# zubair-irshad/NeO-360

Measured on AMD Instinct MI355X. Metric: rays/sec (128 samples/ray) + PSNR vs ref, 640x480, higher is better.
Workload: dtype f32 (fp16-MFMA products of hi/lo-split fp32 operands, fp32 accumulate)

## Files before the change

neo-360_amd/csrc/mlp_tp_hp.hip:

```cpp
#include <hip/hip_fp16.h>

#include <algorithm>
#include <cstdlib>
#include <type_traits>

#include "tp_hp_layout.h"

#ifndef NEO_TP_WPS
#define NEO_TP_WPS 2
#endif
#ifndef NEO_TP_RING
#define NEO_TP_RING 3
#endif
#ifndef NEO_TP_STAGGER_DEFAULT
#define NEO_TP_STAGGER_DEFAULT 0
#endif
#ifndef NEO_TP_XSTREAM
#define NEO_TP_XSTREAM 2
#endif
#ifndef NEO_TP_ABLATE
#define NEO_TP_ABLATE 0
#endif
#define TP_SYNC() __syncthreads()
#ifndef NEO_TP_TRACE
#define NEO_TP_TRACE 0
#endif
#if NEO_TP_TRACE
__device__ unsigned long long g_tp_trace[16];
#define TP_MARK(k) do { const unsigned long long now_ = __builtin_amdgcn_s_memtime(); tr_[k] += now_ - tlast_; tlast_ = now_; } while (0)
#else
#define TP_MARK(k) do { } while (0)
#endif

namespace neo {

namespace {

using namespace hp;
constexpr int RING = NEO_TP_RING;

template <int PE_C, bool CULL = false, bool DENS = false>
__global__ __launch_bounds__(256, NEO_TP_WPS) void k_tp_mlp_hp(TpMlpHDev m, const float* __restrict__ proj, TpScene sc,
                                                             TpViews views, const float* __restrict__ rays_o,
                                                             const float* __restrict__ rays_d,
                                                             const float* __restrict__ viewdirs,
                                                             const float* __restrict__ tvals,
                                                             const float* __restrict__ far_arr, int R, int N, int chunk,
                                                             uint32_t* __restrict__ flags, float4* __restrict__ out, int stagger,
                                                             const float* __restrict__ dirsum) {
    extern __shared__ __attribute__((aligned(16))) float smem[];
    if (stagger > 0 && blockIdx.x >= 256u && blockIdx.x < 512u)
        for (int i = 0; i < stagger; i += 100) __builtin_amdgcn_s_sleep(100);
    _Float16* hbase = reinterpret_cast<_Float16*>(smem + tp::OFF_ACT);
    const HT act{hbase, hbase + TM * 128};
    auto xbuf = [&](int b) { return HT{hbase + b * (2 * TM * 64), hbase + b * (2 * TM * 64) + TM * 64}; };
    auto fbuf = [&](int b) { return smem + tp::OFF_ACT + b * (TM * 64); };
    _Float16* dbase = reinterpret_cast<_Float16*>(smem + tp::OFF_DIR);
    const HT dsm{dbase, dbase + TM * 32};
    const tp::Scratch S = tp::carve(smem);
    int* loc_off = S.loc_off;
    float* loc_w = S.loc_w;
    int* pl_off = S.pl_off;
    float* pl_w = S.pl_w;
    float* cam_enc = S.cam_enc;

    LaneCtx L;
    L.init();
    int tid = threadIdx.x;
    const long P = tp::launch_points<CULL>(sc, R, N);
    const long tile0 = tp::xcd_tile<CULL>(blockIdx.x, (P + TM - 1) / TM) * TM;
    if (tile0 >= P) return;
    const h8* wp = reinterpret_cast<const h8*>(m.wpack);
    constexpr int KSX = ks_x(PE_C);
    constexpr int NPE = PE_C == 3 ? 1 : 2;

#if NEO_TP_TRACE
    unsigned long long tr_[8] = {0, 0, 0, 0, 0, 0, 0, 0}, tlast_ = __builtin_amdgcn_s_memtime();
#endif
    tp::point_setup<PE_C>(S, tid, tile0, P, N, R, chunk, rays_o, rays_d, viewdirs, tvals, far_arr, flags, false, sc.grid_w, sc.grid_first, sc.grid_pw, sc.grid_ph, CULL ? sc.cull_map : nullptr, CULL ? 0 : sc.quad);
    float* dens_w = smem + tp::OFF_DENSW;
    if (tid < 128) dens_w[tid] = m.heads[HD_DW + tid];
    float* lbias_w = smem + tp::LDS_WORDS;
    for (int i = tid; i < 768; i += 256) lbias_w[i] = m.bias[i];
    for (int i = tid; i < HD_RB + 3; i += 256) lbias_w[768 + i] = m.heads[i];
    const float* lbias = lbias_w;
    const float* lheads = lbias_w + 768;
    float* dsum = smem + tp::OFF_DIR;
    TP_SYNC();
    if constexpr (!DENS) {
        const int p = tid >> 2, f0 = (tid & 3) << 3;
        const int dray = __float_as_int(S.vdir_world[p * 4 + 3]);
        const f32x4 s0 = *reinterpret_cast<const f32x4*>(dirsum + (long)dray * 32 + f0);
        const f32x4 s1 = *reinterpret_cast<const f32x4*>(dirsum + (long)dray * 32 + f0 + 4);
#pragma unroll
        for (int j = 0; j < 8; ++j) dsum[p * 32 + ((f0 + j) ^ (p & 31))] = j < 4 ? s0[j] : s1[j - 4];
        TP_SYNC();
    }
    TP_MARK(0);

    f32x16 hsum[2];
#pragma unroll
    for (int r = 0; r < 16; ++r) { hsum[0][r] = 0.f; hsum[1][r] = 0.f; }
    [[maybe_unused]] const int nts_1[1] = {L.wv};
    const int vnt = L.wv & 1, vmt = L.wv >> 1;

#pragma unroll 1
    for (int v = 0; v < sc.nv; ++v) {
        asm volatile("" : "+v"(tid));
        L.lane = tid & 63;
        L.half = L.lane >> 5;
        L.l31 = L.lane & 31;
        L.key = L.lane & 15;
// ... 390 lines not shown
            if constexpr (g == 13) {
                TP_SYNC();
                store_tile_h<true>(y, act, vnt, vmt, L);
            }
            __builtin_amdgcn_sched_barrier(0);
        });
        TP_SYNC();
    }
    {
        const int pt = L.wv * 16 + (L.lane >> 2), part = L.lane & 3;
        [[maybe_unused]] float r = 0.f, g = 0.f, b = 0.f;
        if constexpr (!DENS) {
            const float* wr = lheads + HD_RW;
#pragma unroll
            for (int c = 0; c < 2; ++c) {
                const int chunk_i = part * 2 + ((c + part) & 1);
                const int o = chunk_off<128>(pt, chunk_i);
                const h8 vh = *reinterpret_cast<const h8*>(act.hi + o);
                const h8 vl = *reinterpret_cast<const h8*>(act.lo + o);
#pragma unroll
                for (int e = 0; e < 8; ++e) {
                    const float h = (float)vh[e] + (float)vl[e];
                    r += h * wr[chunk_i * 8 + e];
                    g += h * wr[64 + chunk_i * 8 + e];
                    b += h * wr[128 + chunk_i * 8 + e];
                }
            }
            r += __shfl_xor(r, 1, 64); r += __shfl_xor(r, 2, 64);
            g += __shfl_xor(g, 1, 64); g += __shfl_xor(g, 2, 64);
            b += __shfl_xor(b, 1, 64); b += __shfl_xor(b, 2, 64);
        }
        range_commit(L, m.flags);
        const long gv = tile0 + pt;
        const long gi = tp::launch_point(gv, N, R, CULL ? 0 : sc.quad, sc.grid_w, sc.grid_first, sc.grid_pw, sc.grid_ph);
        if (part == 0 && gv < P) {
            if constexpr (DENS)
                out[gi] = make_float4(0.0f, 0.0f, 0.0f, density_act(raw_sigma));
            else
                out[gi] = make_float4(colour_act(r + lheads[HD_RB]), colour_act(g + lheads[HD_RB + 1]),
                                      colour_act(b + lheads[HD_RB + 2]), density_act(raw_sigma));
        }
    }
#if NEO_TP_TRACE
    TP_MARK(6);
    if (threadIdx.x == 0) {
#pragma unroll
        for (int k = 0; k < 7; ++k) atomicAdd(&g_tp_trace[k], tr_[k]);
        atomicAdd(&g_tp_trace[7], 1ull);
    }
#endif
}

__global__ void k_tp_dirsum(const float* __restrict__ viewdirs, int R, TpViews views, int nv, float* __restrict__ out) {
    const int r = blockIdx.x * blockDim.x + threadIdx.x;
    if (r >= R) return;
    const float dx = viewdirs[r * 3], dy = viewdirs[r * 3 + 1], dz = viewdirs[r * 3 + 2];
    float acc[27];
#pragma unroll
    for (int f = 0; f < 27; ++f) acc[f] = 0.0f;
    for (int v = 0; v < nv; ++v) {
        const float* rot = views.rot[v];
        const float dc[3] = {rot[0] * dx + rot[1] * dy + rot[2] * dz, rot[3] * dx + rot[4] * dy + rot[5] * dz,
                             rot[6] * dx + rot[7] * dy + rot[8] * dz};
#pragma unroll
        for (int a = 0; a < 3; ++a) acc[a] += dc[a];
#pragma unroll
        for (int k = 0; k < 4; ++k)
// ... 122 lines not shown
                          hipStream_t s, int channels, int in_ch, int first_chunk) {
    if (texels <= 0) return;
    const dim3 grid((unsigned)((texels + 63) / 64));
    const f32x4* wx = reinterpret_cast<const f32x4*>(wpack_f32_stage_x);
    if (channels == 128 && in_ch == 512)
        hipLaunchKernelGGL((k_tp_preproject<1, 64>), grid, dim3(256), 0, s, latent_cl, wx, kc_x, texels, proj, first_chunk);
    else if (in_ch == 512)
        hipLaunchKernelGGL((k_tp_preproject<2, 64>), grid, dim3(256), 0, s, latent_cl, wx, kc_x, texels, proj, first_chunk);
    else
        hipLaunchKernelGGL((k_tp_preproject<2, 16>), grid, dim3(256), 0, s, latent_cl, wx, kc_x, texels, proj, first_chunk);
}

void launch_tp_dirsum(const float* viewdirs, int R, const TpViews& views, int nv, float* dirsum, hipStream_t s) {
    if (R <= 0) return;
    hipLaunchKernelGGL(k_tp_dirsum, dim3((unsigned)((R + 255) / 256)), dim3(256), 0, s, viewdirs, R, views, nv, dirsum);
}

void launch_tp_mlp_hp(int input_ch, const TpMlpHDev& m, const float* proj, const TpScene& sc, const TpViews& views,
                      const float* rays_o, const float* rays_d, const float* viewdirs, const float* tvals,
                      const float* far, int R, int N, int chunk, uint32_t* flags, float* out, const float* dirsum,
                      hipStream_t s, bool density_only) {
    const long P = (long)R * N;
    if (P <= 0) return;
    static int stagger = -1;
    if (stagger < 0) {
        const char* e = getenv("NEO_TP_STAGGER");
        stagger = e ? atoi(e) : NEO_TP_STAGGER_DEFAULT;
    }
    static size_t lds_pad = ~size_t(0);
    if (lds_pad == ~size_t(0)) {
        const char* e = getenv("NEO_TP_LDS_PAD");
        lds_pad = e ? (size_t)atol(e) : 0;
    }
    const size_t lds = (tp::LDS_WORDS + 768 + 336) * sizeof(float) + lds_pad;
    if (lds > 65536) {
        (void)hipFuncSetAttribute(reinterpret_cast<const void*>(k_tp_mlp_hp<3>), hipFuncAttributeMaxDynamicSharedMemorySize, (int)lds);
        (void)hipFuncSetAttribute(reinterpret_cast<const void*>(k_tp_mlp_hp<4>), hipFuncAttributeMaxDynamicSharedMemorySize, (int)lds);
        (void)hipFuncSetAttribute(reinterpret_cast<const void*>(k_tp_mlp_hp<4, true>), hipFuncAttributeMaxDynamicSharedMemorySize, (int)lds);
        (void)hipFuncSetAttribute(reinterpret_cast<const void*>(k_tp_mlp_hp<3, true>), hipFuncAttributeMaxDynamicSharedMemorySize, (int)lds);
        (void)hipFuncSetAttribute(reinterpret_cast<const void*>(k_tp_mlp_hp<3, false, true>), hipFuncAttributeMaxDynamicSharedMemorySize, (int)lds);
        (void)hipFuncSetAttribute(reinterpret_cast<const void*>(k_tp_mlp_hp<4, false, true>), hipFuncAttributeMaxDynamicSharedMemorySize, (int)lds);
        (void)hipFuncSetAttribute(reinterpret_cast<const void*>(k_tp_mlp_hp<4, true, true>), hipFuncAttributeMaxDynamicSharedMemorySize, (int)lds);
    }
    const long tiles = tp::xcd_grid((P + TM - 1) / TM);
    const bool dens = density_only && !(sc.cull_map && input_ch == 3);
    if (dens) {
    } else if (!sc.cull_map && input_ch == 3)
        hipLaunchKernelGGL(k_tp_mlp_hp<3>, dim3((unsigned)tiles), dim3(256), lds, s, m, proj, sc, views, rays_o, rays_d,
                           viewdirs, tvals, far, R, N, chunk, flags, reinterpret_cast<float4*>(out), stagger, dirsum);
    else if (sc.cull_map && input_ch != 3)
        hipLaunchKernelGGL((k_tp_mlp_hp<4, true>), dim3((unsigned)tiles), dim3(256), lds, s, m, proj, sc, views, rays_o, rays_d,
                           viewdirs, tvals, far, R, N, chunk, flags, reinterpret_cast<float4*>(out), stagger, dirsum);
    else if (!sc.cull_map)
        hipLaunchKernelGGL(k_tp_mlp_hp<4>, dim3((unsigned)tiles), dim3(256), lds, s, m, proj, sc, views, rays_o, rays_d,
                           viewdirs, tvals, far, R, N, chunk, flags, reinterpret_cast<float4*>(out), stagger, dirsum);
    else
        hipLaunchKernelGGL((k_tp_mlp_hp<3, true>), dim3((unsigned)tiles), dim3(256), lds, s, m, proj, sc, views, rays_o, rays_d,
                           viewdirs, tvals, far, R, N, chunk, flags, reinterpret_cast<float4*>(out), stagger, dirsum);
    if (!dens) return;
    if (!sc.cull_map && input_ch == 3)
        hipLaunchKernelGGL((k_tp_mlp_hp<3, false, true>), dim3((unsigned)tiles), dim3(256), lds, s, m, proj, sc, views, rays_o, rays_d,
                           viewdirs, tvals, far, R, N, chunk, flags, reinterpret_cast<float4*>(out), stagger, dirsum);
    else if (!sc.cull_map)
        hipLaunchKernelGGL((k_tp_mlp_hp<4, false, true>), dim3((unsigned)tiles), dim3(256), lds, s, m, proj, sc, views, rays_o, rays_d,
                           viewdirs, tvals, far, R, N, chunk, flags, reinterpret_cast<float4*>(out), stagger, dirsum);
    else
        hipLaunchKernelGGL((k_tp_mlp_hp<4, true, true>), dim3((unsigned)tiles), dim3(256), lds, s, m, proj, sc, views, rays_o, rays_d,
// ... 5 lines not shown
```

neo-360_amd/csrc/mlp_tp_hpp.hip:

```cpp
#include <hip/hip_fp16.h>

#include <algorithm>
#include <cstdlib>
#include <type_traits>

#include "tp_hp_layout.h"

#ifndef NEO_TPP_WPS
#define NEO_TPP_WPS 2
#endif
#ifndef NEO_TPP_RING
#define NEO_TPP_RING 3
#endif
#ifndef NEO_TPP_XD
#define NEO_TPP_XD 1
#endif
#ifndef NEO_TPP_LD
#define NEO_TPP_LD 4
#endif
#ifndef NEO_TPP_TD
#define NEO_TPP_TD 6
#endif
#define TPP_SYNC() __syncthreads()
#ifndef NEO_TP_TRACE
#define NEO_TP_TRACE 0
#endif
#if NEO_TP_TRACE
__device__ unsigned long long g_tpp_trace[16];
#define TPP_MARK(k) do { const unsigned long long now_ = __builtin_amdgcn_s_memtime(); tr_[k] += now_ - tlast_; tlast_ = now_; } while (0)
#else
#define TPP_MARK(k) do { } while (0)
#endif

namespace neo {

namespace {

using namespace hp;
constexpr int RING = NEO_TPP_RING;

constexpr int PP_OFF_DESC = tp::OFF_DIR + TM * 32;
constexpr int DESC_BLOCK = TM * 4, DESC_W = 5 * DESC_BLOCK;
constexpr int PP_OFF_LIST = PP_OFF_DESC + 2 * DESC_W;
constexpr int LIST_MAX = 18;
constexpr int PP_OFF_CAM = PP_OFF_LIST + 4 * LIST_MAX * 4;
constexpr int PP_OFF_PE = PP_OFF_CAM + TM * 4;
constexpr int PP_OFF_FEAT = PP_OFF_PE + TM * 4;
constexpr int PP_OFF_VDIR = PP_OFF_FEAT + TM * 4;
constexpr int PP_OFF_DENSW = PP_OFF_VDIR + TM * 4;
constexpr int PP_OFF_BIAS = PP_OFF_DENSW + 128;
constexpr int PP_OFF_XPE0 = PP_OFF_BIAS + 768 + 336;
constexpr int PP_LDS_WORDS = PP_OFF_XPE0 + TM * 64;
static_assert(PP_LDS_WORDS * 4 <= 81920, "two workgroups per CU");

struct TpPlaneBase { int texels[3]; };

template <int PE_C, bool CULL = false, bool DENS = false>
__global__ __launch_bounds__(256, NEO_TPP_WPS) void k_tp_mlp_hpp(TpMlpHDev m, const float* __restrict__ proj, TpPlaneBase plb,
                                                               TpScene sc, TpViews views, const float* __restrict__ rays_o,
                                                               const float* __restrict__ rays_d,
                                                               const float* __restrict__ viewdirs,
                                                               const float* __restrict__ tvals,
                                                               const float* __restrict__ far_arr, int R, int N, int chunk,
                                                               uint32_t* __restrict__ flags, float4* __restrict__ out,
                                                               const float* __restrict__ dirsum) {
    extern __shared__ __attribute__((aligned(16))) float smem[];
    _Float16* hbase = reinterpret_cast<_Float16*>(smem + tp::OFF_ACT);
    const HT act{hbase, hbase + TM * 128};
    auto fbuf = [&](int b) { return smem + tp::OFF_ACT + b * (TM * 64); };
    _Float16* xb0 = reinterpret_cast<_Float16*>(smem + PP_OFF_XPE0);
    const HT xpe0{xb0, xb0 + TM * 64};
    _Float16* dbase = reinterpret_cast<_Float16*>(smem + tp::OFF_DIR);
    const HT dsm{dbase, dbase + TM * 32};
    const HT xpe1 = dsm;
    tp::Scratch S;
    S.loc_off = reinterpret_cast<int*>(smem + PP_OFF_DESC);
    S.pl_off = S.loc_off + DESC_BLOCK;
    S.loc_w = smem + PP_OFF_DESC + DESC_W;
    S.pl_w = S.loc_w + DESC_BLOCK;
    S.cam_enc = smem + PP_OFF_CAM;
    S.pe_world = smem + PP_OFF_PE;
    S.feat_world = smem + PP_OFF_FEAT;
    S.vdir_world = smem + PP_OFF_VDIR;
    [[maybe_unused]] int* loc_off = S.loc_off;
    float* loc_w = S.loc_w;
    [[maybe_unused]] int* pl_off = S.pl_off;

    LaneCtx L;
    L.init();
    int tid = threadIdx.x;
    const long P = tp::launch_points<CULL>(sc, R, N);
    const long tile0 = tp::xcd_tile<CULL>(blockIdx.x, (P + TM - 1) / TM) * TM;
    if (tile0 >= P) return;
    const h8* wp = reinterpret_cast<const h8*>(m.wpack);
    constexpr int KSX = ks_x(PE_C);
    constexpr int KSP = pe_ksteps(PE_C);
    constexpr int NPE = PE_C == 3 ? 1 : 2;

#if NEO_TP_TRACE
    unsigned long long tr_[8] = {0, 0, 0, 0, 0, 0, 0, 0}, tlast_ = __builtin_amdgcn_s_memtime();
#endif
    tp::point_setup<PE_C>(S, tid, tile0, P, N, R, chunk, rays_o, rays_d, viewdirs, tvals, far_arr, flags, false, sc.grid_w, sc.grid_first, sc.grid_pw, sc.grid_ph, CULL ? sc.cull_map : nullptr, CULL ? 0 : sc.quad);
    float* dens_w = smem + PP_OFF_DENSW;
    if (tid < 128) dens_w[tid] = m.heads[HD_DW + tid];
    if (tid < DESC_BLOCK) {
        S.loc_off[4 * DESC_BLOCK + tid] = 0;
        S.loc_w[4 * DESC_BLOCK + tid] = 0.0f;
    }
    float* lbias_w = smem + PP_OFF_BIAS;
    for (int i = tid; i < 768; i += 256) lbias_w[i] = m.bias[i];
    for (int i = tid; i < HD_RB + 3; i += 256) lbias_w[768 + i] = m.heads[i];
    const float* lbias = lbias_w;
    const float* lheads = lbias_w + 768;
    TPP_SYNC();

    f32x16 hsum[2];
#pragma unroll
    for (int r = 0; r < 16; ++r) { hsum[0][r] = 0.f; hsum[1][r] = 0.f; }
    const int vnt = L.wv & 1, vmt = L.wv >> 1;

    TPP_MARK(0);
#pragma unroll 1
    for (int v = 0; v < sc.nv; ++v) {
        asm volatile("" : "+v"(tid));
        L.lane = tid & 63;
        L.half = L.lane >> 5;
        L.l31 = L.lane & 31;
        L.key = L.lane & 15;
        const float* rot = views.rot[v];
        const float* trn = views.trans[v];
        tp::view_descriptors<PROJ_TEXEL_BYTES, false, PROJ_TEXEL_BYTES>(S, L, sc, rot, trn, v, [](int, int, float) {},
                                                                        L.wv == 0 ? 0 : plb.texels[L.wv == 0 ? 0 : L.wv - 1]);
        {
            const int row = tid & 63, q = tid >> 6;
            const float ex = S.pe_world[row * 4], ey = S.pe_world[row * 4 + 1], ez = S.pe_world[row * 4 + 2];
            f32x4 xv;
            xv[0] = (rot[0] * ex + rot[1] * ey + rot[2] * ez) + trn[0];
            xv[1] = (rot[3] * ex + rot[4] * ey + rot[5] * ez) + trn[1];
            xv[2] = (rot[6] * ex + rot[7] * ey + rot[8] * ez) + trn[2];
            xv[3] = S.pe_world[row * 4 + 3];
            auto pe_chunk = [&](auto ldh, const HT& buf, int pstage, int hf) __attribute__((always_inline)) {
                constexpr int LDH = decltype(ldh)::value;
                const int chs = hf * 4 + q;
                const int ch = pstage * 8 + chs;
                float f[8];
                h8 vh, vl;
                if (ch * 4 < 10 * PE_C) {
#pragma unroll
                    for (int jj = 0; jj < 4; ++jj) {
                        if (PE_C == 3 && jj >= 2 && ch == 7) {
                            f[2 * jj] = jj == 2 ? xv[0] : xv[2];
                            f[2 * jj + 1] = jj == 2 ? xv[1] : 0.0f;
                            range_see(L, f[2 * jj]); range_see(L, f[2 * jj + 1]);
                            continue;
                        }
                        float x;
                        int oct;
                        if constexpr (PE_C == 4) {
                            x = xv[jj];
                            oct = ch;
                        } else {
                            const int p = ch * 4 + jj;
                            oct = p / 3;
                            const int a = p - 3 * oct;
                            x = a == 0 ? xv[0] : a == 1 ? xv[1] : xv[2];
                        }
// ... 71 lines not shown
                }
#pragma unroll
                for (int nt = 0; nt < 2; ++nt)
#pragma unroll
                    for (int mt = 0; mt < 2; ++mt) {
                        accx[nt][mt] = NEO_MFMA_H_LH(wl[kp % XS][nt], bh[mt], accx[nt][mt]);
                        accx[nt][mt] = NEO_MFMA_H_HL(wh[kp % XS][nt], bl[mt], accx[nt][mt]);
                        accx[nt][mt] = NEO_MFMA_H(wh[kp % XS][nt], bh[mt], accx[nt][mt]);
                    }
                load_wk(std::integral_constant<int, kp + XD>());
            };
            auto consume_chunk = [&](auto cc) __attribute__((always_inline)) {
                constexpr int c = decltype(cc)::value;
                const float* buf = fbuf(c & 1);
#pragma unroll
                for (int mt = 0; mt < 2; ++mt)
#pragma unroll
                    for (int gg = 0; gg < 2; ++gg) {
                        const int row = mt * 32 + L.l31;
                        const int piece = L.wv * 4 + gg * 2 + L.half;
                        const f32x4 val = *reinterpret_cast<const f32x4*>(buf + row * 64 + ((piece ^ (row & 15)) << 2));
                        constexpr int g0 = 2 * (c & 1);
#pragma unroll
                        for (int e = 0; e < 4; ++e) accx[c >> 1][mt][4 * (g0 + gg) + e] += val[e];
                    }
            };
            static_assert(RING == 3 && LIST_MAX % RING == 0, "the work-list pipeline is written for a ring of three");
            int n_p;
            bool any_w;
            const int4* list;
            {
                int4* mylist = reinterpret_cast<int4*>(smem + PP_OFF_LIST) + L.wv * LIST_MAX;
                unsigned am = 0;
#pragma unroll
                for (int mp = 0; mp < 4; ++mp) {
                    const f32x4 w = *reinterpret_cast<const f32x4*>(loc_w + (mp * TM + L.lane) * 4);
                    const unsigned long long z = __ballot(w[0] != 0.0f || w[1] != 0.0f || w[2] != 0.0f || w[3] != 0.0f);
#pragma unroll
                    for (int q = 0; q < 4; ++q) am |= (((z >> (16 * q)) & 0xFFFFull) != 0ull ? 1u : 0u) << (4 * q + mp);
                }
                any_w = am != 0u;
#pragma unroll
                for (int q = 0; q < 4; ++q)
                    if (((am >> (4 * q)) & 0xFu) == 0u) am |= 1u << (4 * q);
                const int n = __builtin_popcount(am);
                n_p = ((n + RING - 1) / RING) * RING;
                {
                    const int b = L.lane;
                    const bool real = b < 16 && ((am >> b) & 1u);
                    const bool pad = b - 32 >= n && b - 32 < n_p;
                    if (real || pad) {
                        int4 rec;
                        int at = b - 32;
                        if (real) {
                            const int q = b >> 2, mp = b & 3;
                            const unsigned grp = (am >> (4 * q)) & 0xFu;
                            rec.x = (mp * TM + 16 * q) * 16;
                            rec.y = 16 * q;
                            rec.z = (grp & ((1u << mp) - 1u)) == 0u ? 0 : 0x3f800000;
                            rec.w = (grp >> (mp + 1)) == 0u ? 1 : 0;
                            at = __builtin_popcount(am & ((1u << b) - 1u));
                        } else {
                            rec.x = 4 * DESC_BLOCK * 4;
                            rec.y = 0;
                            rec.z = 0x3f800000;
                            rec.w = 0;
// ... 206 lines not shown
            if constexpr (g == 13) {
                TPP_SYNC();
                store_tile_h<true>(y, act, vnt, vmt, L);
            }
            __builtin_amdgcn_sched_barrier(0);
        });
        TPP_SYNC();
    }
    {
        const int pt = L.wv * 16 + (L.lane >> 2), part = L.lane & 3;
        [[maybe_unused]] float r = 0.f, g = 0.f, b = 0.f;
        if constexpr (!DENS) {
            const float* wr = lheads + HD_RW;
#pragma unroll
            for (int c = 0; c < 2; ++c) {
                const int chunk_i = part * 2 + ((c + part) & 1);
                const int o = chunk_off<128>(pt, chunk_i);
                const h8 vh = *reinterpret_cast<const h8*>(act.hi + o);
                const h8 vl = *reinterpret_cast<const h8*>(act.lo + o);
#pragma unroll
                for (int e = 0; e < 8; ++e) {
                    const float h = (float)vh[e] + (float)vl[e];
                    r += h * wr[chunk_i * 8 + e];
                    g += h * wr[64 + chunk_i * 8 + e];
                    b += h * wr[128 + chunk_i * 8 + e];
                }
            }
            r += __shfl_xor(r, 1, 64); r += __shfl_xor(r, 2, 64);
            g += __shfl_xor(g, 1, 64); g += __shfl_xor(g, 2, 64);
            b += __shfl_xor(b, 1, 64); b += __shfl_xor(b, 2, 64);
        }
        range_commit(L, m.flags);
        const long gv = tile0 + pt;
        const long gi = tp::launch_point(gv, N, R, CULL ? 0 : sc.quad, sc.grid_w, sc.grid_first, sc.grid_pw, sc.grid_ph);
        if (part == 0 && gv < P) {
            if constexpr (DENS)
                out[gi] = make_float4(0.0f, 0.0f, 0.0f, density_act(raw_sigma));
            else
                out[gi] = make_float4(colour_act(r + lheads[HD_RB]), colour_act(g + lheads[HD_RB + 1]),
                                      colour_act(b + lheads[HD_RB + 2]), density_act(raw_sigma));
        }
    }
#if NEO_TP_TRACE
    TPP_MARK(5);
    if (threadIdx.x == 0) {
#pragma unroll
        for (int k = 0; k < 6; ++k) atomicAdd(&g_tpp_trace[k], tr_[k]);
        atomicAdd(&g_tpp_trace[7], 1ull);
    }
#endif
}

}

#if NEO_TP_TRACE
extern "C" void neo_debug_tpp_trace(unsigned long long* host16, int reset) {
    (void)hipDeviceSynchronize();
    (void)hipMemcpyFromSymbol(host16, HIP_SYMBOL(g_tpp_trace), sizeof(unsigned long long) * 16);
    if (reset) {
        unsigned long long z[16] = {0};
        (void)hipMemcpyToSymbol(HIP_SYMBOL(g_tpp_trace), z, sizeof(z));
    }
}
#endif

void launch_tp_mlp_hpp(int input_ch, const TpMlpHDev& m, const float* proj_all, const long plane_base_texels[3],
                       const TpScene& sc, const TpViews& views, const float* rays_o, const float* rays_d, const float* viewdirs,
// ... 49 lines not shown
```

neo-360_amd/csrc/tp_common.h:

```cpp
#pragma once
#include "kernels.h"
#include "mfma_tile.h"
#include "point_order.h"

namespace neo {
namespace tp {

constexpr int TM = 64;

constexpr int OFF_ACT = 0;
constexpr int OFF_DIR = OFF_ACT + TM * 128;
constexpr int OFF_LOC_OFF = OFF_DIR + TM * 32;
constexpr int OFF_LOC_W = OFF_LOC_OFF + TM * 4;
constexpr int OFF_PL_OFF = OFF_LOC_W + TM * 4;
constexpr int OFF_PL_W = OFF_PL_OFF + 3 * TM * 4;
constexpr int OFF_CAM = OFF_PL_W + 3 * TM * 4;
constexpr int OFF_PE = OFF_CAM + TM * 4;
constexpr int OFF_FEAT = OFF_PE + TM * 4;
constexpr int OFF_VDIR = OFF_FEAT + TM * 4;
constexpr int OFF_DENSW = OFF_VDIR + TM * 4;
constexpr int LDS_WORDS = OFF_DENSW + 128;

constexpr int XCDS = 8;
template <bool COMPACT = false>
// ... 70 lines not shown
#pragma unroll
    for (int e = 0; e < 4; ++e) {
        float a = __builtin_fmaf(tap[0][e], w[0], acc[e]);
        a = __builtin_fmaf(tap[1][e], w[1], a);
        a = __builtin_fmaf(tap[2][e], w[2], a);
        a = __builtin_fmaf(tap[3][e], w[3], a);
        v[e] = a;
    }
    return v;
}

__device__ __forceinline__ f32x4 load_tap(const float* __restrict__ base, uint32_t off) {
    return *reinterpret_cast<const f32x4*>(reinterpret_cast<const char*>(base) + off);
}

template <int C>
__device__ __forceinline__ float pe_feature(const float* x, int f) {
    if (f < C) return x[f];
    const int g = f - C;
    if (g < 10 * C) return sin_cw(ldexpf(x[g % C], g / C));
    const int h = g - 10 * C;
    if (h < 10 * C) return sin_cw(ldexpf(x[h % C], h / C) + HALF_PI_F32);
    return 0.0f;
}



template <int PE_C>
__device__ __forceinline__ void point_setup_row(const Scratch& S, int tid, long tile0, long P, int N, int R, int chunk,
                                                const float* __restrict__ rays_o, const float* __restrict__ rays_d,
                                                const float* __restrict__ viewdirs, const float* __restrict__ tvals,
                                                const float* __restrict__ far_arr, uint32_t* __restrict__ flags,
                                                bool t_shared = false, int grid_w = 0, long grid_first = 0, int pw = 3, int ph = 3,
                                                const int* __restrict__ cull_map = nullptr, int quad = 0) {
    float* pe_world = S.pe_world;
    float* feat_world = S.feat_world;
    float* vdir_world = S.vdir_world;
    {
        long g = tile0 + tid;
        if (g >= P) g = P - 1;
        g = launch_point(g, N, R, quad, grid_w, grid_first, pw, ph);
        const int row = (int)(g / N);
        const int s = (int)(g - (long)row * N);
        const int ray = cull_map ? cull_map[row] : row;
        const int c0 = (ray / chunk) * chunk;
        const int bc = min(chunk, R - c0);
        const int gl = (ray - c0) * N + s;
        const int dray = c0 + gl % bc;
        const float tv = tvals[t_shared ? (long)s : g];
        float o[3], d[3];
#pragma unroll
        for (int a = 0; a < 3; ++a) { o[a] = rays_o[ray * 3 + a]; d[a] = rays_d[ray * 3 + a]; }
        if (PE_C == 3) {
#pragma unroll
            for (int a = 0; a < 3; ++a) {
                const float x = o[a] + tv * d[a];
                pe_world[tid * 4 + a] = x;
                feat_world[tid * 4 + a] = x;
            }
            pe_world[tid * 4 + 3] = 0.0f;
        } else {
            const float far = far_arr[ray];
            const float dd = d[0] * d[0] + d[1] * d[1] + d[2] * d[2];
            const float d1 = -(d[0] * o[0] + d[1] * o[1] + d[2] * o[2]) / dd;
            float pm[3];
#pragma unroll
            for (int a = 0; a < 3; ++a) pm[a] = o[a] + d1 * d[a];
            const float rmid = sqrtf(pm[0] * pm[0] + pm[1] * pm[1] + pm[2] * pm[2]);
            const float inv_len = 1.0f / sqrtf(dd);
            const float margin = 1.0f - rmid * rmid;
            if (!(margin >= 0.0f)) atomicOr(flags, 1u);
            const float d2 = sqrtf(margin) * inv_len;
            float ps[3];
#pragma unroll
            for (int a = 0; a < 3; ++a) ps[a] = o[a] + (d1 + d2) * d[a];
            float ax[3] = {o[1] * ps[2] - o[2] * ps[1], o[2] * ps[0] - o[0] * ps[2], o[0] * ps[1] - o[1] * ps[0]};
            const float an = sqrtf(ax[0] * ax[0] + ax[1] * ax[1] + ax[2] * ax[2]);
#pragma unroll
            for (int a = 0; a < 3; ++a) ax[a] = ax[a] / an;
            const float ang = asinf(rmid) - asinf(rmid * tv);
            const float ca = cosf(ang), sa = sinf(ang);
            const float cr[3] = {ax[1] * ps[2] - ax[2] * ps[1], ax[2] * ps[0] - ax[0] * ps[2], ax[0] * ps[1] - ax[1] * ps[0]};
            const float dotp = ax[0] * ps[0] + ax[1] * ps[1] + ax[2] * ps[2];
            float tn[3];
#pragma unroll
            for (int a = 0; a < 3; ++a) tn[a] = ps[a] * ca + cr[a] * sa + ax[a] * dotp * (1.0f - ca);
            const float nn = sqrtf(tn[0] * tn[0] + tn[1] * tn[1] + tn[2] * tn[2]) + 1e-10f;
            const float tl = far * (1.0f - tv) + 3.0f * tv;
#pragma unroll
            for (int a = 0; a < 3; ++a) {
                pe_world[tid * 4 + a] = tn[a] / nn;
                feat_world[tid * 4 + a] = o[a] + tl * d[a];
            }
            pe_world[tid * 4 + 3] = tv;
        }
#pragma unroll
        for (int a = 0; a < 3; ++a) vdir_world[tid * 4 + a] = viewdirs[dray * 3 + a];
        vdir_world[tid * 4 + 3] = __int_as_float(dray);
    }
}

template <int PE_C>
__device__ __forceinline__ void point_setup(const Scratch& S, int tid, long tile0, long P, int N, int R, int chunk,
                                            const float* __restrict__ rays_o, const float* __restrict__ rays_d,
                                            const float* __restrict__ viewdirs, const float* __restrict__ tvals,
                                            const float* __restrict__ far_arr, uint32_t* __restrict__ flags,
                                            bool t_shared = false, int grid_w = 0, long grid_first = 0, int pw = 3, int ph = 3,
                                            const int* __restrict__ cull_map = nullptr, int quad = 0) {
    if (tid < TM)
        point_setup_row<PE_C>(S, tid, tile0, P, N, R, chunk, rays_o, rays_d, viewdirs, tvals, far_arr, flags, t_shared, grid_w, grid_first, pw, ph, cull_map, quad);
}

template <int LOC_TEXEL_BYTES = 2048, bool DIRS = true, int PL_TEXEL_BYTES = 128 * 4, class PutDir>
__device__ __forceinline__ void view_descriptors(const Scratch& S, const LaneCtx& L, const TpScene& sc,
                                                 const float* rot, const float* trn, int v, PutDir put_dir,
                                                 int pl_base_texels = 0) {
    int* loc_off = S.loc_off; float* loc_w = S.loc_w; int* pl_off = S.pl_off; float* pl_w = S.pl_w;
    float* cam_enc = S.cam_enc; const float* pe_world = S.pe_world; const float* feat_world = S.feat_world;
    const float* vdir_world = S.vdir_world;
        {
            const int p = L.lane;
            const float fx = feat_world[p * 4], fy = feat_world[p * 4 + 1], fz = feat_world[p * 4 + 2];
            const float cx_ = (rot[0] * fx + rot[1] * fy + rot[2] * fz) + trn[0];
            const float cy_ = (rot[3] * fx + rot[4] * fy + rot[5] * fz) + trn[1];
            const float cz_ = (rot[6] * fx + rot[7] * fy + rot[8] * fz) + trn[2];
            TapSet t;
            int* dst_off;
            float* dst_w;
            int base, texel_bytes;
            if (L.wv == 0) {
                const float den = cz_ + 1e-9f;
                const float u = (-cx_ / den) * sc.focal + sc.cx;
                const float w_ = (-cy_ / den) * (sc.fy_sign * sc.focal) + sc.cy;
                t = bilinear_taps(u * sc.sx - 1.0f, w_ * sc.sy - 1.0f, sc.Wf, sc.Hf);
                dst_off = loc_off; dst_w = loc_w;
                base = v * sc.Hf * sc.Wf;
                texel_bytes = LOC_TEXEL_BYTES;
                const float ex = pe_world[p * 4], ey = pe_world[p * 4 + 1], ez = pe_world[p * 4 + 2];
                cam_enc[p * 4 + 0] = (rot[0] * ex + rot[1] * ey + rot[2] * ez) + trn[0];
                cam_enc[p * 4 + 1] = (rot[3] * ex + rot[4] * ey + rot[5] * ez) + trn[1];
                cam_enc[p * 4 + 2] = (rot[6] * ex + rot[7] * ey + rot[8] * ez) + trn[2];
                cam_enc[p * 4 + 3] = pe_world[p * 4 + 3];
            } else {
                const float ga = L.wv == 3 ? cy_ : cx_;
                const float gb = L.wv == 2 ? cy_ : cz_;
                t = bilinear_taps(ga, gb, sc.Wp, sc.Hp);
                dst_off = pl_off + (L.wv - 1) * TM * 4; dst_w = pl_w + (L.wv - 1) * TM * 4;
                base = v * sc.Hp * sc.Wp + pl_base_texels;
                texel_bytes = PL_TEXEL_BYTES;
            }
#pragma unroll
            for (int k = 0; k < 4; ++k) {
                dst_off[p * 4 + k] = (int)((uint32_t)(base + t.off[k]) * (uint32_t)texel_bytes);
                dst_w[p * 4 + k] = t.w[k];
            }
            if constexpr (!DIRS) return;
            const float dx = vdir_world[p * 4], dy = vdir_world[p * 4 + 1], dz = vdir_world[p * 4 + 2];
            const float dc[3] = {rot[0] * dx + rot[1] * dy + rot[2] * dz, rot[3] * dx + rot[4] * dy + rot[5] * dz,
                                 rot[6] * dx + rot[7] * dy + rot[8] * dz};
#pragma unroll
            for (int a = 0; a < 3; ++a) {
                float sn, cs;
                enc_pair(dc[a], L.wv, sn, cs);
                put_dir(p, 3 + L.wv * 3 + a, sn);
                put_dir(p, 15 + L.wv * 3 + a, cs);
            }
            if (L.wv == 0) {
#pragma unroll
                for (int a = 0; a < 3; ++a) put_dir(p, a, dc[a]);
            }
            if (L.wv == 1) {
#pragma unroll
                for (int f = 27; f < 32; ++f) put_dir(p, f, 0.0f);
            }
        }
}

}
}
```

Before: 523,300.

## Cache point indices in LDS, precompute tap-weight bits, redistribute PE sincos across waves

Stores each row's launch-point index in LDS during point setup so the output store reuses it instead of recomputing launch_point. In the hpp kernel it also ballots whether each point's bilinear taps have nonzero weight and stores per-wave bit masks, replacing the per-lane reads of loc_w when building the active mask. It also adds a static schedule that spreads the positional-encoding sin/cos octaves across the four waves and writes the split fp16 hi/lo values straight into the LDS tiles. The cost is extra LDS (point records and weight bits) and more complex, wave-specialised code paths that could add register pressure.

Result: faster. 529,100, median of 6 (+1.1%).

```diff
diff --git a/neo-360_amd/csrc/mlp_tp_hp.hip b/neo-360_amd/csrc/mlp_tp_hp.hip
--- a/neo-360_amd/csrc/mlp_tp_hp.hip
+++ b/neo-360_amd/csrc/mlp_tp_hp.hip
@@ -20,6 +20,9 @@
 #endif
 #ifndef NEO_TP_ABLATE
 #define NEO_TP_ABLATE 0
+#endif
+#ifndef NEO_TP_ROW_POINT
+#define NEO_TP_ROW_POINT 1
 #endif
 #define TP_SYNC() __syncthreads()
 #ifndef NEO_TP_TRACE
@@ -38,6 +41,9 @@
 
 using namespace hp;
 constexpr int RING = NEO_TP_RING;
+constexpr int HP_OFF_POINT = tp::LDS_WORDS + 768 + 336;
+constexpr int HP_LDS_WORDS = HP_OFF_POINT + (NEO_TP_ROW_POINT ? TM * 2 : 0);
+static_assert(HP_OFF_POINT % 2 == 0, "8-byte records");
 
 template <int PE_C, bool CULL = false, bool DENS = false>
 __global__ __launch_bounds__(256, NEO_TP_WPS) void k_tp_mlp_hp(TpMlpHDev m, const float* __restrict__ proj, TpScene sc,
@@ -77,7 +83,9 @@
 #if NEO_TP_TRACE
     unsigned long long tr_[8] = {0, 0, 0, 0, 0, 0, 0, 0}, tlast_ = __builtin_amdgcn_s_memtime();
 #endif
-    tp::point_setup<PE_C>(S, tid, tile0, P, N, R, chunk, rays_o, rays_d, viewdirs, tvals, far_arr, flags, false, sc.grid_w, sc.grid_first, sc.grid_pw, sc.grid_ph, CULL ? sc.cull_map : nullptr, CULL ? 0 : sc.quad);
+    [[maybe_unused]] long* row_point = reinterpret_cast<long*>(smem + HP_OFF_POINT);
+    tp::point_setup<PE_C>(S, tid, tile0, P, N, R, chunk, rays_o, rays_d, viewdirs, tvals, far_arr, flags, false, sc.grid_w, sc.grid_first, sc.grid_pw, sc.grid_ph, CULL ? sc.cull_map : nullptr, CULL ? 0 : sc.quad,
+                          NEO_TP_ROW_POINT ? row_point : nullptr);
     float* dens_w = smem + tp::OFF_DENSW;
     if (tid < 128) dens_w[tid] = m.heads[HD_DW + tid];
     float* lbias_w = smem + tp::LDS_WORDS;
@@ -534,7 +542,9 @@
         }
         range_commit(L, m.flags);
         const long gv = tile0 + pt;
-        const long gi = tp::launch_point(gv, N, R, CULL ? 0 : sc.quad, sc.grid_w, sc.grid_first, sc.grid_pw, sc.grid_ph);
+        long gi;
+        if constexpr (NEO_TP_ROW_POINT != 0) gi = row_point[pt];
+        else gi = tp::launch_point(gv, N, R, CULL ? 0 : sc.quad, sc.grid_w, sc.grid_first, sc.grid_pw, sc.grid_ph);
         if (part == 0 && gv < P) {
             if constexpr (DENS)
                 out[gi] = make_float4(0.0f, 0.0f, 0.0f, density_act(raw_sigma));
@@ -723,7 +733,7 @@
         const char* e = getenv("NEO_TP_LDS_PAD");
         lds_pad = e ? (size_t)atol(e) : 0;
     }
-    const size_t lds = (tp::LDS_WORDS + 768 + 336) * sizeof(float) + lds_pad;
+    const size_t lds = HP_LDS_WORDS * sizeof(float) + lds_pad;
     if (lds > 65536) {
         (void)hipFuncSetAttribute(reinterpret_cast<const void*>(k_tp_mlp_hp<3>), hipFuncAttributeMaxDynamicSharedMemorySize, (int)lds);
         (void)hipFuncSetAttribute(reinterpret_cast<const void*>(k_tp_mlp_hp<4>), hipFuncAttributeMaxDynamicSharedMemorySize, (int)lds);
diff --git a/neo-360_amd/csrc/mlp_tp_hpp.hip b/neo-360_amd/csrc/mlp_tp_hpp.hip
--- a/neo-360_amd/csrc/mlp_tp_hpp.hip
+++ b/neo-360_amd/csrc/mlp_tp_hpp.hip
@@ -4,6 +4,7 @@
 #include <cstdlib>
 #include <type_traits>
 
+#include "pe_schedule.h"
 #include "tp_hp_layout.h"
 
 #ifndef NEO_TPP_WPS
@@ -20,6 +21,9 @@
 #endif
 #ifndef NEO_TPP_TD
 #define NEO_TPP_TD 6
+#endif
+#ifndef NEO_TPP_FRONT
+#define NEO_TPP_FRONT 7
 #endif
 #define TPP_SYNC() __syncthreads()
 #ifndef NEO_TP_TRACE
@@ -50,7 +54,10 @@
 constexpr int PP_OFF_DENSW = PP_OFF_VDIR + TM * 4;
 constexpr int PP_OFF_BIAS = PP_OFF_DENSW + 128;
 constexpr int PP_OFF_XPE0 = PP_OFF_BIAS + 768 + 336;
-constexpr int PP_LDS_WORDS = PP_OFF_XPE0 + TM * 64;
+constexpr int PP_OFF_POINT = PP_OFF_XPE0 + TM * 64;
+constexpr int PP_OFF_WBITS = PP_OFF_POINT + TM * 2;
+constexpr int PP_LDS_WORDS = PP_OFF_WBITS + 4;
+static_assert(PP_OFF_POINT % 2 == 0 && PP_OFF_WBITS % 4 == 0, "8-byte records, one 16-byte read");
 static_assert(PP_LDS_WORDS * 4 <= 81920, "two workgroups per CU");
 
 struct TpPlaneBase { int texels[3]; };
@@ -100,7 +107,12 @@
 #if NEO_TP_TRACE
     unsigned long long tr_[8] = {0, 0, 0, 0, 0, 0, 0, 0}, tlast_ = __builtin_amdgcn_s_memtime();
 #endif
-    tp::point_setup<PE_C>(S, tid, tile0, P, N, R, chunk, rays_o, rays_d, viewdirs, tvals, far_arr, flags, false, sc.grid_w, sc.grid_first, sc.grid_pw, sc.grid_ph, CULL ? sc.cull_map : nullptr, CULL ? 0 : sc.quad);
+    constexpr bool PE_TILE = PE_C == 4 && (NEO_TPP_FRONT & 1) != 0;
+    constexpr bool ROW_POINT = (NEO_TPP_FRONT & 2) != 0, WBITS = (NEO_TPP_FRONT & 4) != 0;
+    [[maybe_unused]] long* row_point = reinterpret_cast<long*>(smem + PP_OFF_POINT);
+    [[maybe_unused]] unsigned* wbits = reinterpret_cast<unsigned*>(smem + PP_OFF_WBITS);
+    tp::point_setup<PE_C>(S, tid, tile0, P, N, R, chunk, rays_o, rays_d, viewdirs, tvals, far_arr, flags, false, sc.grid_w, sc.grid_first, sc.grid_pw, sc.grid_ph, CULL ? sc.cull_map : nullptr, CULL ? 0 : sc.quad,
+                          ROW_POINT ? row_point : nullptr);
     float* dens_w = smem + PP_OFF_DENSW;
     if (tid < 128) dens_w[tid] = m.heads[HD_DW + tid];
     if (tid < DESC_BLOCK) {
@@ -113,6 +125,50 @@
     const float* lbias = lbias_w;
     const float* lheads = lbias_w + 768;
     TPP_SYNC();
+    [[maybe_unused]] _Float16* const pe_h = reinterpret_cast<_Float16*>(smem);
+    [[maybe_unused]] auto pe_at = [&](auto firstc, int row, int pos) __attribute__((always_inline)) {
+        if constexpr (decltype(firstc)::value) return PP_OFF_XPE0 * 2 + chunk_off<64>(row, pos >> 3) + (pos & 7);
+        else return tp::OFF_DIR * 2 + chunk_off<32>(row, (pos - 64) >> 3) + (pos & 7);
+    };
+    [[maybe_unused]] constexpr std::true_type PE_FIRST{};
+    [[maybe_unused]] constexpr std::false_type PE_SECOND{};
+    [[maybe_unused]] constexpr int LO0 = TM * 64, LO1 = TM * 32;
+    if constexpr (PE_TILE) {
+        namespace ps = pe_sched;
+        const int row = tid & 63, q = L.wv;
+        const float tv = S.pe_world[row * 4 + 3];
+        static_for<0, ps::TILE_SLOTS>([&](auto sl) {
+            constexpr int slot = decltype(sl)::value;
+            constexpr bool first = ps::WAVES * slot + ps::WAVES <= 8;
+            if (slot < ps::OCTAVES / ps::WAVES || slot < ps::tile_pairs(q)) {
+                const int oct = ps::tile_octave(q, slot);
+                float sn, cs;
+                sincos_pair(ldexpf(tv, oct), sn, cs);
+                h2 h, l;
+                split2(sn, cs, h, l);
+                const int o = pe_at(std::bool_constant<first>(), row, ps::pair_pos(oct, 3));
+                *reinterpret_cast<h2*>(pe_h + o) = h;
+                *reinterpret_cast<h2*>(pe_h + o + (first ? LO0 : LO1)) = l;
+            }
+        });
+        if (q == ps::TILE_IDENT_WAVE) {
+            range_see(L, tv);
+            h2 h, l;
+            split2(tv, 0.0f, h, l);
+            const int o = pe_at(PE_SECOND, row, ps::IDENT_POS + 3);
+            pe_h[o] = h[0];
+            pe_h[o + LO1] = l[0];
+            const h4 z = {0, 0, 0, 0};
+            *reinterpret_cast<h4*>(pe_h + o + 1) = z;
+            *reinterpret_cast<h4*>(pe_h + o + 1 + LO1) = z;
+        }
+        if (q == ps::TILE_PAD_WAVE) {
+            const int o = pe_at(PE_SECOND, row, ps::PAD_POS + 4);
+            const h8 z = {0, 0, 0, 0, 0, 0, 0, 0};
+            *reinterpret_cast<h8*>(pe_h + o) = z;
+            *reinterpret_cast<h8*>(pe_h + o + LO1) = z;
+        }
+    }
 
     f32x16 hsum[2];
 #pragma unroll
@@ -129,9 +185,71 @@
         L.key = L.lane & 15;
         const float* rot = views.rot[v];
         const float* trn = views.trans[v];
-        tp::view_descriptors<PROJ_TEXEL_BYTES, false, PROJ_TEXEL_BYTES>(S, L, sc, rot, trn, v, [](int, int, float) {},
-                                                                        L.wv == 0 ? 0 : plb.texels[L.wv == 0 ? 0 : L.wv - 1]);
-        {
+        const bool weighted =
+            tp::view_descriptors<PROJ_TEXEL_BYTES, false, PROJ_TEXEL_BYTES>(S, L, sc, rot, trn, v, [](int, int, float) {},
+                                                                            L.wv == 0 ? 0 : plb.texels[L.wv == 0 ? 0 : L.wv - 1]);
+        if constexpr (WBITS) {
+            const unsigned long long z = __ballot(weighted);
+            unsigned bits = 0;
+#pragma unroll
+            for (int g = 0; g < 4; ++g) bits |= (((z >> (16 * g)) & 0xFFFFull) != 0ull ? 1u : 0u) << g;
+            if (L.lane == 0) wbits[L.wv] = bits;
+        }
+        if constexpr (PE_TILE) {
+            namespace ps = pe_sched;
+            const int row = tid & 63;
+            int q = L.wv;
+            asm volatile("" : "+s"(q));
+            const float ex = S.pe_world[row * 4], ey = S.pe_world[row * 4 + 1], ez = S.pe_world[row * 4 + 2];
+            float xv[3];
+            xv[0] = (rot[0] * ex + rot[1] * ey + rot[2] * ez) + trn[0];
+            xv[1] = (rot[3] * ex + rot[4] * ey + rot[5] * ez) + trn[1];
+            xv[2] = (rot[6] * ex + rot[7] * ey + rot[8] * ez) + trn[2];
+            asm("" : "+v"(xv[0]), "+v"(xv[1]), "+v"(xv[2]));
+            static_for<0, ps::VIEW_LOW_SLOTS / 3>([&](auto kc) {
+                constexpr int k = decltype(kc)::value;
+                const int oct = ps::view_octave(q, 3 * k);
+                h2 h[3], l[3];
+#pragma unroll
+                for (int a = 0; a < 3; ++a) {
+                    static_assert(ps::view_coord(0, 3 * k) == 0 && ps::view_coord(3, 3 * k + 1) == 1 && ps::view_coord(1, 3 * k + 2) == 2);
+                    float sn, cs;
+                    sincos_pair(ldexpf(xv[a], oct), sn, cs);
+                    split2(sn, cs, h[a], l[a]);
+                }
+                const int o = pe_at(PE_FIRST, row, ps::pair_pos(oct, 0));
+                *reinterpret_cast<h4*>(pe_h + o) = h4{h[0][0], h[0][1], h[1][0], h[1][1]};
+                *reinterpret_cast<h2*>(pe_h + o + 4) = h[2];
+                *reinterpret_cast<h4*>(pe_h + o + LO0) = h4{l[0][0], l[0][1], l[1][0], l[1][1]};
+                *reinterpret_cast<h2*>(pe_h + o + 4 + LO0) = l[2];
+            });
+            static_for<ps::VIEW_LOW_SLOTS, ps::VIEW_SLOTS>([&](auto sl) {
+                constexpr int slot = decltype(sl)::value;
+                if (slot < ps::VIEW_PAIRS / ps::WAVES || slot < ps::view_pairs(q)) {
+                    const int oct = ps::view_octave(q, slot), a = ps::view_coord(q, slot);
+                    const unsigned m0 = a == 0 ? ~0u : 0u, m1 = a == 1 ? ~0u : 0u, m2 = a == 2 ? ~0u : 0u;
+                    const float x = __uint_as_float((__float_as_uint(xv[0]) & m0) | (__float_as_uint(xv[1]) & m1) | (__float_as_uint(xv[2]) & m2));
+                    float sn, cs;
+                    sincos_pair(ldexpf(x, oct), sn, cs);
+                    h2 h, l;
+                    split2(sn, cs, h, l);
+                    const int o = pe_at(PE_SECOND, row, ps::pair_pos(oct, a));
+                    *reinterpret_cast<h2*>(pe_h + o) = h;
+                    *reinterpret_cast<h2*>(pe_h + o + LO1) = l;
+                }
+            });
+            if (q == ps::VIEW_IDENT_WAVE) {
+                range_see(L, xv[0]); range_see(L, xv[1]); range_see(L, xv[2]);
+                h2 h, l, hz, lz;
+                split2(xv[0], xv[1], h, l);
+                split2(xv[2], 0.0f, hz, lz);
+                const int o = pe_at(PE_SECOND, row, ps::IDENT_POS);
+                *reinterpret_cast<h2*>(pe_h + o) = h;
+                *reinterpret_cast<h2*>(pe_h + o + LO1) = l;
+                pe_h[o + 2] = hz[0];
+                pe_h[o + 2 + LO1] = lz[0];
+            }
+        } else {
             const int row = tid & 63, q = tid >> 6;
             const float ex = S.pe_world[row * 4], ey = S.pe_world[row * 4 + 1], ez = S.pe_world[row * 4 + 2];
             f32x4 xv;
@@ -269,6 +387,15 @@
             {
                 int4* mylist = reinterpret_cast<int4*>(smem + PP_OFF_LIST) + L.wv * LIST_MAX;
                 unsigned am = 0;
+                if constexpr (WBITS) {
+                    const uint4 wb = *reinterpret_cast<const uint4*>(wbits);
+                    const unsigned w4[4] = {wb.x, wb.y, wb.z, wb.w};
+#pragma unroll
+                    for (int mp = 0; mp < 4; ++mp)
+#pragma unroll
+                        for (int q = 0; q < 4; ++q) am |= ((w4[mp] >> q) & 1u) << (4 * q + mp);
+                    am = __builtin_amdgcn_readfirstlane(am);
+                } else
 #pragma unroll
                 for (int mp = 0; mp < 4; ++mp) {
                     const f32x4 w = *reinterpret_cast<const f32x4*>(loc_w + (mp * TM + L.lane) * 4);
@@ -541,7 +668,9 @@
         }
         range_commit(L, m.flags);
         const long gv = tile0 + pt;
-        const long gi = tp::launch_point(gv, N, R, CULL ? 0 : sc.quad, sc.grid_w, sc.grid_first, sc.grid_pw, sc.grid_ph);
+        long gi;
+        if constexpr (ROW_POINT) gi = row_point[pt];
+        else gi = tp::launch_point(gv, N, R, CULL ? 0 : sc.quad, sc.grid_w, sc.grid_first, sc.grid_pw, sc.grid_ph);
         if (part == 0 && gv < P) {
             if constexpr (DENS)
                 out[gi] = make_float4(0.0f, 0.0f, 0.0f, density_act(raw_sigma));
diff --git a/neo-360_amd/csrc/pe_schedule.h b/neo-360_amd/csrc/pe_schedule.h
--- /dev/null
+++ b/neo-360_amd/csrc/pe_schedule.h
@@ -0,0 +1,38 @@
+#pragma once
+
+#if defined(__HIPCC__) || defined(__CUDACC__)
+#define NEO_PS_HD __host__ __device__ __forceinline__
+#else
+#define NEO_PS_HD inline
+#endif
+
+namespace neo {
+namespace pe_sched {
+
+constexpr int WAVES = 4, OCTAVES = 10, COORDS = 4, WIDTH = 96;
+constexpr int IDENT_POS = 2 * OCTAVES * COORDS;
+constexpr int PAD_POS = IDENT_POS + COORDS;
+constexpr int VIEW_PAIRS = OCTAVES * (COORDS - 1);
+constexpr int VIEW_SLOTS = (VIEW_PAIRS + WAVES - 1) / WAVES;
+constexpr int VIEW_LOW_SLOTS = 2 * (COORDS - 1);
+constexpr int TILE_SLOTS = (OCTAVES + WAVES - 1) / WAVES;
+constexpr int VIEW_IDENT_WAVE = 3;
+constexpr int TILE_IDENT_WAVE = 2;
+constexpr int TILE_PAD_WAVE = 3;
+
+NEO_PS_HD constexpr int pair_pos(int oct, int coord) { return 2 * (oct * COORDS + coord); }
+
+NEO_PS_HD constexpr int view_pairs(int wave) { return VIEW_LOW_SLOTS + 1 + (wave < VIEW_PAIRS - WAVES * (VIEW_LOW_SLOTS + 1) ? 1 : 0); }
+NEO_PS_HD constexpr int view_high(int wave, int slot) { return (slot - VIEW_LOW_SLOTS) * WAVES + wave; }
+NEO_PS_HD constexpr int view_octave(int wave, int slot) {
+    return slot < VIEW_LOW_SLOTS ? 2 * wave + slot / (COORDS - 1) : 2 * WAVES + view_high(wave, slot) / (COORDS - 1);
+}
+NEO_PS_HD constexpr int view_coord(int wave, int slot) {
+    return slot < VIEW_LOW_SLOTS ? slot % (COORDS - 1) : view_high(wave, slot) % (COORDS - 1);
+}
+
+NEO_PS_HD constexpr int tile_pairs(int wave) { return OCTAVES / WAVES + (wave < OCTAVES % WAVES ? 1 : 0); }
+NEO_PS_HD constexpr int tile_octave(int wave, int slot) { return wave + WAVES * slot; }
+
+}
+}
diff --git a/neo-360_amd/csrc/tp_common.h b/neo-360_amd/csrc/tp_common.h
--- a/neo-360_amd/csrc/tp_common.h
+++ b/neo-360_amd/csrc/tp_common.h
@@ -126,7 +126,8 @@
                                                 const float* __restrict__ viewdirs, const float* __restrict__ tvals,
                                                 const float* __restrict__ far_arr, uint32_t* __restrict__ flags,
                                                 bool t_shared = false, int grid_w = 0, long grid_first = 0, int pw = 3, int ph = 3,
-                                                const int* __restrict__ cull_map = nullptr, int quad = 0) {
+                                                const int* __restrict__ cull_map = nullptr, int quad = 0,
+                                                long* row_point = nullptr) {
     float* pe_world = S.pe_world;
     float* feat_world = S.feat_world;
     float* vdir_world = S.vdir_world;
@@ -134,6 +135,7 @@
         long g = tile0 + tid;
         if (g >= P) g = P - 1;
         g = launch_point(g, N, R, quad, grid_w, grid_first, pw, ph);
+        if (row_point) row_point[tid] = g;
         const int row = (int)(g / N);
         const int s = (int)(g - (long)row * N);
         const int ray = cull_map ? cull_map[row] : row;
@@ -200,13 +202,14 @@
                                             const float* __restrict__ viewdirs, const float* __restrict__ tvals,
                                             const float* __restrict__ far_arr, uint32_t* __restrict__ flags,
                                             bool t_shared = false, int grid_w = 0, long grid_first = 0, int pw = 3, int ph = 3,
-                                            const int* __restrict__ cull_map = nullptr, int quad = 0) {
+                                            const int* __restrict__ cull_map = nullptr, int quad = 0,
+                                            long* row_point = nullptr) {
     if (tid < TM)
-        point_setup_row<PE_C>(S, tid, tile0, P, N, R, chunk, rays_o, rays_d, viewdirs, tvals, far_arr, flags, t_shared, grid_w, grid_first, pw, ph, cull_map, quad);
+        point_setup_row<PE_C>(S, tid, tile0, P, N, R, chunk, rays_o, rays_d, viewdirs, tvals, far_arr, flags, t_shared, grid_w, grid_first, pw, ph, cull_map, quad, row_point);
 }
 
 template <int LOC_TEXEL_BYTES = 2048, bool DIRS = true, int PL_TEXEL_BYTES = 128 * 4, class PutDir>
-__device__ __forceinline__ void view_descriptors(const Scratch& S, const LaneCtx& L, const TpScene& sc,
+__device__ __forceinline__ bool view_descriptors(const Scratch& S, const LaneCtx& L, const TpScene& sc,
                                                  const float* rot, const float* trn, int v, PutDir put_dir,
                                                  int pl_base_texels = 0) {
     int* loc_off = S.loc_off; float* loc_w = S.loc_w; int* pl_off = S.pl_off; float* pl_w = S.pl_w;
@@ -248,7 +251,8 @@
                 dst_off[p * 4 + k] = (int)((uint32_t)(base + t.off[k]) * (uint32_t)texel_bytes);
                 dst_w[p * 4 + k] = t.w[k];
             }
-            if constexpr (!DIRS) return;
+            const bool weighted = t.w[0] != 0.0f || t.w[1] != 0.0f || t.w[2] != 0.0f || t.w[3] != 0.0f;
+            if constexpr (!DIRS) return weighted;
             const float dx = vdir_world[p * 4], dy = vdir_world[p * 4 + 1], dz = vdir_world[p * 4 + 2];
             const float dc[3] = {rot[0] * dx + rot[1] * dy + rot[2] * dz, rot[3] * dx + rot[4] * dy + rot[5] * dz,
                                  rot[6] * dx + rot[7] * dy + rot[8] * dz};
@@ -267,6 +271,7 @@
 #pragma unroll
                 for (int f = 27; f < 32; ++f) put_dir(p, f, 0.0f);
             }
+            return weighted;
         }
 }
 
```
